# yezhen17/3DIoUMatch

Hardware: AMD Instinct MI355X
Metric: scenes/sec train-step (ScanNet 40k pts, 256 proposals) (higher is better)
Workload: dtype f32

## Files before the change

3dioumatch_amd/csrc/mlp_bwd_fused.hip:

```cpp
#include "common.h"
#include "mlp_operand.h"
#include "mlp_bwd_x6.h"

#ifndef MLP_LIN4_OCC
#define MLP_LIN4_OCC 1
#endif

namespace {

template <int MB, int KB, int KBD, int NB, int PMODE, int QMODE, int OCC, bool STATS, bool DGRAD = true,
          bool X6 = false>
__global__ void __launch_bounds__(256, OCC)
gemm_bwd_fused_kernel(int k_total, int r, int total_chunks, int chunks_per_cloud, int xyz,
                      OperandB opp, OperandB opq, const float *__restrict__ w,
                      float *__restrict__ dq, float *__restrict__ part,
                      float *__restrict__ stats_part) {
  constexpr int M = 32 * MB, KP = 32 * KB, TN = 32 * NB;
  constexpr int LDP = M + 1, LDQ = KP + 1;
  constexpr int TPR = TN / 16;
  constexpr int RPP = 256 / TPR;
  constexpr int PP = (M + RPP - 1) / RPP, QP = (KP + RPP - 1) / RPP;
  constexpr int WMB = MB >= 4 ? MB / 4 : 1;
  constexpr int WKB = MB >= 4 ? KB : KB * MB / 4;
  static_assert(MB >= 4 ? MB % 4 == 0 : (MB == 2 && KB % 2 == 0), "dW blocks must split over 4 waves");
  constexpr int DK = KBD >= 4 ? KBD / 4 : 1;
  constexpr int DN = KBD >= 4 ? NB : 1;
  static_assert(KBD >= 4 ? KBD % 4 == 0 : (KBD == 2 && NB == 2), "dQ blocks must split over 4 waves");
  constexpr int DU = 4, DG = DGRAD ? (X6 ? M / 16 : (M / 2) / DU) : 0;
  constexpr int WU = WMB * WKB >= 4 ? 1 : 2, WG = X6 ? TN / 16 : (TN / 2) / WU;
  constexpr int NS = 4 * (PP + QP), NG = DG + WG;

  __shared__ float Ps[2][TN * LDP];
  __shared__ float Qs[2][TN * LDQ];
  static_assert(DGRAD || !STATS, "the sums come from the dQ blocks");
  static_assert(!STATS || QMODE == OP_BNRELU || QMODE == OP_LIN4,
                "the sums are those of a BatchNorm+ReLU layer below");
  constexpr bool QLIN = QMODE == OP_LIN4;
  static_assert(!QLIN || (STATS && KB * 32 == 64), "recomputed rows: the 64-channel layer only");
  constexpr bool TF = QLIN;
  static_assert(!TF || X6, "the T form is instantiated in the bf16 form only");
  constexpr bool RAWQ = STATS;
  constexpr int SROWS = STATS ? 32 * KBD : 1;
  __shared__ float4 Rc[SROWS];
  __shared__ float4 X4s[TF ? 2 : 1][TF ? TN : 1];
  __shared__ float Wx[3 * M];
  __shared__ float red[8 * 3 * 32];

  const int tid = threadIdx.x, lane = tid & 63, wave = tid >> 6;
  const int l31 = lane & 31, lhi = lane >> 5;
  const int seg_row = tid / TPR, seg_c = (tid % TPR) * 16;
  OperandB P = opp, Q = opq;

  static_assert(M % RPP == 0, "whole passes over the P rows");
  RowCoef pc[PP], qc[QP];
  bool q_ok[QP];
  size_t p_lane[PP], q_lane[QP];
#pragma unroll
  for (int p = 0; p < PP; ++p) {
    pc[p] = load_row_coef<PMODE>(P, seg_row + p * RPP, true);
    p_lane[p] = (size_t)(seg_row + p * RPP) * r + seg_c;
  }
#pragma unroll
  for (int q = 0; q < QP; ++q) {
    const int row = seg_row + q * RPP;
    q_ok[q] = row < k_total;
    qc[q] = load_row_coef<QLIN ? OP_BNRELU : QMODE>(Q, q_ok[q] ? row : k_total - 1, true);
    q_lane[q] = QLIN ? (size_t)seg_c : (size_t)(q_ok[q] ? row : k_total - 1) * r + seg_c;
  }
  float4 qw[QP];
#pragma unroll
  for (int q = 0; q < QP; ++q) {
    const int row = seg_row + q * RPP;
    qw[q] = QLIN && row < k_total ? *reinterpret_cast<const float4 *>(Q.lin_w + (size_t)row * 4)
                                 : make_float4(0.f, 0.f, 0.f, 0.f);
  }
  if (STATS) {
    for (int t = tid; t < SROWS; t += 256)
      Rc[t] = make_float4(Q.scale[t], Q.shift[t], Q.mean[t], Q.invstd[t]);
  }
  float fsc[WKB], fsh[WKB];
#pragma unroll
  for (int j = 0; j < WKB; ++j) {
    const int kb = MB >= 4 ? j : (wave / MB) + (4 / MB) * j;
    const int row = kb * 32 + l31;
    fsc[j] = RAWQ && row < k_total ? Q.scale[row] : 1.f;
    fsh[j] = RAWQ && row < k_total ? Q.shift[row] : 0.f;
  }
  const int lane_g = PMODE == OP_POOLDY ? seg_c / P.ns : 0;
  const int lane_s = PMODE == OP_POOLDY ? seg_c % P.ns : 0;

  float wreg[DK][DGRAD ? M / 2 : 1];
#pragma unroll
  for (int e = 0; e < (DGRAD ? DK : 0); ++e) {
    const int kbd = KBD >= 4 ? wave * DK + e : (wave >> 1);
    const float *wc = w + xyz + 32 * kbd + l31;
#pragma unroll
    for (int s = 0; s < M / 2; ++s)
      wreg[e][s] = wc[(size_t)(X6 ? 16 * (s >> 3) + 8 * lhi + (s & 7) : 2 * s + lhi) * k_total];
  }
  for (int t = tid; t < 3 * M; t += 256) Wx[t] = DGRAD && xyz ? w[(size_t)(t % M) * k_total + t / M] : 0.f;

  f32x16 accW[WMB][WKB];
#pragma unroll
  for (int i = 0; i < WMB; ++i)
#pragma unroll
    for (int j = 0; j < WKB; ++j)
#pragma unroll
      for (int q = 0; q < 16; ++q) accW[i][j][q] = 0.f;

  const int per = (total_chunks + (int)gridDim.x - 1) / (int)gridDim.x;
  const int c_lo = (int)blockIdx.x * per;
  const int c_hi = c_lo + per < total_chunks ? c_lo + per : total_chunks;

  float4 px[PP][4], pd[PP][4], qx[QP][4][QLIN ? 4 : 1];
  int pwin[PP];
  float pdp[PP];
#pragma unroll
  for (int p = 0; p < PP; ++p) {
    pwin[p] = -1; pdp[p] = 0.f;
#pragma unroll
    for (int i = 0; i < 4; ++i) { px[p][i] = make_float4(0.f, 0.f, 0.f, 0.f); pd[p][i] = px[p][i]; }
  }
#pragma unroll
  for (int q = 0; q < QP; ++q)
#pragma unroll
    for (int i = 0; i < 4; ++i)
#pragma unroll
      for (int cc = 0; cc < (QLIN ? 4 : 1); ++cc) qx[q][i][cc] = make_float4(0.f, 0.f, 0.f, 0.f);

  struct ChunkAt { size_t p, q, grp; int s0; };
  auto chunk_at = [&](int c) {
    const int b = c / chunks_per_cloud;
    const int col0 = (c - b * chunks_per_cloud) * TN;
    ChunkAt at;
    at.p = (size_t)b * M * r + col0;
    at.q = (size_t)b * (QLIN ? 4 : k_total) * r + col0;
    at.grp = 0; at.s0 = 0;
    if (PMODE == OP_POOLDY) {
      const int g0 = col0 / P.ns;
      at.grp = (size_t)b * M * P.groups + g0;
      at.s0 = col0 - g0 * P.ns;
    }
    return at;
  };
  auto fetch_slice = [&](int sl, const ChunkAt &at) {
    if (sl < 4 * PP) {
      const int p = sl >> 2, i = sl & 3;
      px[p][i] = *reinterpret_cast<const float4 *>(P.x + at.p + p_lane[p] + 4 * i);
      if (PMODE == OP_DY) {
        pd[p][i] = *reinterpret_cast<const float4 *>(P.dz + at.p + p_lane[p] + 4 * i);
      } else if (PMODE == OP_POOLDY && i == 3) {
        const size_t gi = at.grp + (size_t)(seg_row + p * RPP) * P.groups + lane_g;
        pwin[p] = P.argmax[gi] - (at.s0 + lane_s);
        pdp[p] = P.dz[gi];
      }
    } else {
      const int q = (sl - 4 * PP) >> 2, i = (sl - 4 * PP) & 3;
      if constexpr (QLIN) {
#pragma unroll
        for (int cc = 0; cc < 4; ++cc)
          qx[q][i][cc] = *reinterpret_cast<const float4 *>(Q.x + at.q + (size_t)cc * r + q_lane[q] + 4 * i);
      } else {
        qx[q][i][0] = *reinterpret_cast<const float4 *>(Q.x + at.q + q_lane[q] + 4 * i);
      }
    }
  };
  auto stage_slice = [&](int sl, int buf) {
    if (sl < 4 * PP) {
      const int p = sl >> 2, i = sl & 3;
      const int row = seg_row + p * RPP;
      const float xv[4] = {px[p][i].x, px[p][i].y, px[p][i].z, px[p][i].w};
      const float dv[4] = {pd[p][i].x, pd[p][i].y, pd[p][i].z, pd[p][i].w};
#pragma unroll
      for (int e = 0; e < 4; ++e) {
        const float dz = PMODE == OP_POOLDY ? (4 * i + e == pwin[p] ? pdp[p] : 0.f) : dv[e];
        Ps[buf][(seg_c + 4 * i + e) * LDP + row] = transform<PMODE>(xv[e], dz, pc[p]);
      }
    } else {
      const int q = (sl - 4 * PP) >> 2, i = (sl - 4 * PP) & 3;
      const int row = seg_row + q * RPP;
      if (q * RPP >= KP) return;
      if (KP % RPP != 0 && row >= KP) return;
      float xv[4];
      if constexpr (QLIN) {
        const float c0[4] = {qx[q][i][0].x, qx[q][i][0].y, qx[q][i][0].z, qx[q][i][0].w};
        const float c1[4] = {qx[q][i][1].x, qx[q][i][1].y, qx[q][i][1].z, qx[q][i][1].w};
        const float c2[4] = {qx[q][i][2].x, qx[q][i][2].y, qx[q][i][2].z, qx[q][i][2].w};
        const float c3[4] = {qx[q][i][3].x, qx[q][i][3].y, qx[q][i][3].z, qx[q][i][3].w};
#pragma unroll
        for (int e = 0; e < 4; ++e) xv[e] = lin4(qw[q], c0[e], c1[e], c2[e], c3[e]);
        if (TF && row == 0) {
#pragma unroll
          for (int e = 0; e < 4; ++e) X4s[buf][seg_c + 4 * i + e] = make_float4(c0[e], c1[e], c2[e], c3[e]);
        }
      } else {
        xv[0] = qx[q][i][0].x; xv[1] = qx[q][i][0].y; xv[2] = qx[q][i][0].z; xv[3] = qx[q][i][0].w;
      }
#pragma unroll
      for (int e = 0; e < 4; ++e)
        Qs[buf][(seg_c + 4 * i + e) * LDQ + row] =
            q_ok[q] ? (RAWQ ? xv[e] : transform<QLIN ? OP_BNRELU : QMODE>(xv[e], 0.f, qc[q])) : 0.f;
    }
  };

  constexpr int SQ = (STATS && !TF) ? 16 : 1;
  float st1[DK][SQ], st2[DK][SQ];
  float gx[TF ? DK : 1][4];
#pragma unroll
  for (int e = 0; e < (TF ? DK : 1); ++e)
#pragma unroll
    for (int k = 0; k < 4; ++k) gx[e][k] = 0.f;
  float4 trc[TF ? DK : 1];
#pragma unroll
  for (int e = 0; e < (TF ? DK : 1); ++e) {
    const int row = 32 * (KBD >= 4 ? wave * DK + e : (wave >> 1)) + l31;
    trc[e] = TF ? make_float4(Q.scale[row], Q.shift[row], Q.mean[row], Q.invstd[row]) : make_float4(0.f, 0.f, 0.f, 0.f);
  }
#pragma unroll
  for (int e = 0; e < DK; ++e)
#pragma unroll
    for (int q = 0; q < SQ; ++q) { st1[e][q] = 0.f; st2[e][q] = 0.f; }

  if (c_lo < c_hi) {
    const ChunkAt first = chunk_at(c_lo), second = chunk_at(c_lo + 1 < c_hi ? c_lo + 1 : c_lo);
#pragma unroll
    for (int sl = 0; sl < NS; ++sl) fetch_slice(sl, first);
#pragma unroll
    for (int sl = 0; sl < NS; ++sl) {
      stage_slice(sl, 0);
      fetch_slice(sl, second);
    }
  }
  __syncthreads();

  for (int c = c_lo; c < c_hi; ++c) {
    const int cur = (c - c_lo) & 1;
    const float *Pc = Ps[cur], *Qc = Qs[cur];
    const ChunkAt ahead = chunk_at(c + 2 < c_hi ? c + 2 : c_hi - 1);
    auto between = [&](int g) {
#if !defined(BWDF_ABL) || BWDF_ABL != 1
#pragma unroll
      for (int sl = g * NS / NG; sl < (g + 1) * NS / NG; ++sl) {
        stage_slice(sl, cur ^ 1);
        fetch_slice(sl, ahead);
      }
#endif
    };
    const int b = c / chunks_per_cloud;
    const int col0 = (c - b * chunks_per_cloud) * TN;

    f32x16 accD[DK][DN];
    if (DGRAD) {
#pragma unroll
      for (int e = 0; e < DK; ++e)
#pragma unroll
        for (int n = 0; n < DN; ++n)
#pragma unroll
          for (int q = 0; q < 16; ++q) accD[e][n][q] = 0.f;
      if constexpr (X6) {
        float bp8[DN][8];
        auto frag8 = [&](int g) {
#pragma unroll
          for (int n = 0; n < DN; ++n) {
            const int nb = KBD >= 4 ? n : (wave & 1);
#pragma unroll
            for (int j = 0; j < 8; ++j) bp8[n][j] = Pc[(nb * 32 + l31) * LDP + 16 * g + 8 * lhi + j];
          }
        };
        frag8(0);
#pragma unroll
        for (int g = 0; g < DG; ++g) {
          Split3 sb[DN];
#pragma unroll
          for (int n = 0; n < DN; ++n) sb[n] = split3(bp8[n]);
          if (g + 1 < DG) frag8(g + 1);
#pragma unroll
          for (int e = 0; e < DK; ++e) {
            float w8[8];
#pragma unroll
            for (int j = 0; j < 8; ++j) w8[j] = wreg[e][g * 8 + j];
            const Split3 sa = split3(w8);
#pragma unroll
            for (int n = 0; n < DN; ++n) {
              if constexpr (TF) mfma_x6(accD[e][n], sb[n], sa);
              else mfma_x6(accD[e][n], sa, sb[n]);
            }
          }
          between(g);
        }
      } else {
      float bp[2][DU][DN];
      auto frag = [&](int g, float (&dst)[DU][DN]) {
#pragma unroll
        for (int u = 0; u < DU; ++u)
#pragma unroll
          for (int n = 0; n < DN; ++n) {
            const int nb = KBD >= 4 ? n : (wave & 1);
            dst[u][n] = Pc[(nb * 32 + l31) * LDP + 2 * (g * DU + u) + lhi];
          }
      };
      frag(0, bp[0]);
#pragma unroll
      for (int g = 0; g < DG; ++g) {
        if (g + 1 < DG) frag(g + 1, bp[(g + 1) & 1]);
        __builtin_amdgcn_sched_barrier(0);
#pragma unroll
        for (int u = 0; u < DU; ++u)
#pragma unroll
          for (int e = 0; e < DK; ++e)
#pragma unroll
            for (int n = 0; n < DN; ++n)
              accD[e][n] = __builtin_amdgcn_mfma_f32_32x32x2f32(wreg[e][g * DU + u], bp[g & 1][u][n],
                                                                accD[e][n], 0, 0, 0);
        between(g);
        __builtin_amdgcn_sched_barrier(0);
      }
      }
#pragma unroll
      for (int e = 0; e < (TF ? 0 : DK); ++e) {
        const int kbd = KBD >= 4 ? wave * DK + e : (wave >> 1);
#pragma unroll
        for (int n = 0; n < DN; ++n) {
          const int nb = KBD >= 4 ? n : (wave & 1);
          float *dst = dq + ((size_t)b * k_total + xyz + 32 * kbd + 4 * lhi) * r + col0 + nb * 32 + l31;
#pragma unroll
          for (int q = 0; q < 16; ++q)
            __builtin_nontemporal_store(accD[e][n][q], &dst[(size_t)((q & 3) + 8 * (q >> 2)) * r]);
        }
      }
    }

    auto stats_row = [&](int q) {
      const int ro = (q & 3) + 8 * (q >> 2);
      if constexpr (TF) {
#pragma unroll
        for (int e = 0; e < DK; ++e) {
          const int kbd = KBD >= 4 ? wave * DK + e : (wave >> 1);
#pragma unroll
          for (int n = 0; n < DN; ++n) {
            const int nb = KBD >= 4 ? n : (wave & 1);
            const int col = nb * 32 + 4 * lhi + ro;
            const float yv = Qc[col * LDQ + 32 * kbd + l31];
            const float g = __fmaf_rn(yv, trc[e].x, trc[e].y) > 0.f ? accD[e][n][q] : 0.f;
            st1[e][0] += g;
            st2[e][0] = __fmaf_rn(g, (yv - trc[e].z) * trc[e].w, st2[e][0]);
            const float4 xc = X4s[cur][col];
            gx[e][0] = __fmaf_rn(g, xc.x, gx[e][0]);
            gx[e][1] = __fmaf_rn(g, xc.y, gx[e][1]);
            gx[e][2] = __fmaf_rn(g, xc.z, gx[e][2]);
            gx[e][3] = __fmaf_rn(g, xc.w, gx[e][3]);
          }
        }
        return;
      }
#pragma unroll
      for (int e = 0; e < DK; ++e) {
        const int kbd = KBD >= 4 ? wave * DK + e : (wave >> 1);
        const float4 rc = Rc[32 * kbd + 4 * lhi + ro];
#pragma unroll
        for (int n = 0; n < DN; ++n) {
          const int nb = KBD >= 4 ? n : (wave & 1);
          const float yv = Qc[(nb * 32 + l31) * LDQ + 32 * kbd + 4 * lhi + ro];
          const float g = __fmaf_rn(yv, rc.x, rc.y) > 0.f ? accD[e][n][q] : 0.f;
          st1[e][STATS ? q : 0] += g;
          st2[e][STATS ? q : 0] = __fmaf_rn(g, (yv - rc.z) * rc.w, st2[e][STATS ? q : 0]);
        }
      }
    };
    if constexpr (X6) {
      float qraw[8];
      auto qfrag = [&](int g, int j) {
        const int kb = MB >= 4 ? j : (wave / MB) + (4 / MB) * j;
#pragma unroll
        for (int jj = 0; jj < 8; ++jj) {
          const float raw = Qc[(16 * g + 8 * lhi + jj) * LDQ + kb * 32 + l31];
          qraw[jj] = RAWQ ? fmaxf(__fmaf_rn(raw, fsc[j], fsh[j]), 0.f) : raw;
        }
      };
#pragma unroll
      for (int g = 0; g < WG; ++g) {
        Split3 sp[WMB];
#pragma unroll
        for (int i = 0; i < WMB; ++i) {
          const int mb = MB >= 4 ? wave + 4 * i : wave % MB;
          float praw[8];
#pragma unroll
          for (int jj = 0; jj < 8; ++jj) praw[jj] = Pc[(16 * g + 8 * lhi + jj) * LDP + mb * 32 + l31];
          sp[i] = split3(praw);
        }
        qfrag(g, 0);
#pragma unroll
        for (int j = 0; j < WKB; ++j) {
          const Split3 sq = split3(qraw);
          if (j + 1 < WKB) qfrag(g, j + 1);
#pragma unroll
          for (int i = 0; i < WMB; ++i) mfma_x6(accW[i][j], sp[i], sq);
        }
        between(DG + g);
        if (STATS) {
#pragma unroll
          for (int q = g * 16 / WG; q < (g + 1) * 16 / WG; ++q) stats_row(q);
        }
      }
    } else {
      float ap[2][WU][WMB], bq[2][WU][WKB];
      auto frag = [&](int g, float (&a)[WU][WMB], float (&bb)[WU][WKB]) {
#pragma unroll
        for (int u = 0; u < WU; ++u) {
          const int n = 2 * (g * WU + u) + lhi;
#pragma unroll
          for (int i = 0; i < WMB; ++i) {
            const int mb = MB >= 4 ? wave + 4 * i : wave % MB;
            a[u][i] = Pc[n * LDP + mb * 32 + l31];
          }
#pragma unroll
          for (int j = 0; j < WKB; ++j) {
            const int kb = MB >= 4 ? j : (wave / MB) + (4 / MB) * j;
            const float raw = Qc[n * LDQ + kb * 32 + l31];
            bb[u][j] = RAWQ ? fmaxf(__fmaf_rn(raw, fsc[j], fsh[j]), 0.f) : raw;
          }
        }
      };
      frag(0, ap[0], bq[0]);
#pragma unroll
      for (int g = 0; g < WG; ++g) {
        if (g + 1 < WG) frag(g + 1, ap[(g + 1) & 1], bq[(g + 1) & 1]);
        __builtin_amdgcn_sched_barrier(0);
#pragma unroll
        for (int u = 0; u < WU; ++u)
#pragma unroll
          for (int i = 0; i < WMB; ++i)
#pragma unroll
            for (int j = 0; j < WKB; ++j)
              accW[i][j] = __builtin_amdgcn_mfma_f32_32x32x2f32(ap[g & 1][u][i], bq[g & 1][u][j],
                                                                accW[i][j], 0, 0, 0);
        between(DG + g);
        if (STATS) {
#pragma unroll
          for (int q = g * 16 / WG; q < (g + 1) * 16 / WG; ++q) stats_row(q);
        }
        __builtin_amdgcn_sched_barrier(0);
      }
    }

    if (DGRAD && NB == 1 && xyz) {
      const int n = tid & 31, g8 = tid >> 5;
      float s0 = 0.f, s1 = 0.f, s2 = 0.f;
#pragma unroll 4
      for (int mm = g8 * (M / 8); mm < (g8 + 1) * (M / 8); ++mm) {
        const float pv = Pc[n * LDP + mm];
        s0 = __fmaf_rn(pv, Wx[mm], s0);
        s1 = __fmaf_rn(pv, Wx[M + mm], s1);
        s2 = __fmaf_rn(pv, Wx[2 * M + mm], s2);
      }
      red[(g8 * 3 + 0) * 32 + n] = s0;
      red[(g8 * 3 + 1) * 32 + n] = s1;
      red[(g8 * 3 + 2) * 32 + n] = s2;
      __syncthreads();
      if (tid < 96) {
        const int kx = tid >> 5;
        float t = 0.f;
#pragma unroll
        for (int g = 0; g < 8; ++g) t += red[(g * 3 + kx) * 32 + n];
        dq[((size_t)b * k_total + kx) * r + col0 + n] = t;
      }
    }
    __syncthreads();
  }

  if constexpr (TF) {
    constexpr int PPW = KBD >= 4 ? 1 : 2;
    const int parts = (int)gridDim.x * PPW;
    const int pidx = (int)blockIdx.x * PPW + (KBD >= 4 ? 0 : (wave & 1));
#pragma unroll
    for (int e = 0; e < DK; ++e) {
      const int row = 32 * (KBD >= 4 ? wave * DK + e : (wave >> 1)) + l31;
      float a1 = st1[e][0], a2 = st2[e][0];
      a1 += __shfl_xor(a1, 32, kWave);
      a2 += __shfl_xor(a2, 32, kWave);
      float g4[4];
#pragma unroll
      for (int k = 0; k < 4; ++k) g4[k] = gx[e][k] + __shfl_xor(gx[e][k], 32, kWave);
      if (lhi == 0) {
        if (stats_part != nullptr) {
          stats_part[((size_t)row * parts + pidx) * 2] = a1;
          stats_part[((size_t)row * parts + pidx) * 2 + 1] = a2;
        }
        *reinterpret_cast<float4 *>(dq + ((size_t)pidx * k_total + row) * 4) = make_float4(g4[0], g4[1], g4[2], g4[3]);
      }
    }
  } else if (STATS && stats_part != nullptr) {
    constexpr int PPW = KBD >= 4 ? 1 : 2;
    const int parts = (int)gridDim.x * PPW;
    const int pidx = (int)blockIdx.x * PPW + (KBD >= 4 ? 0 : (wave & 1));
#pragma unroll
    for (int e = 0; e < DK; ++e) {
      const int kbd = KBD >= 4 ? wave * DK + e : (wave >> 1);
#pragma unroll
      for (int q = 0; q < SQ; ++q) {
        float a1 = st1[e][q], a2 = st2[e][q];
#pragma unroll
        for (int off = 1; off < 32; off <<= 1) {
          a1 += __shfl_xor(a1, off, kWave);
          a2 += __shfl_xor(a2, off, kWave);
        }
        if (l31 == 0) {
          const int row = 32 * kbd + 4 * lhi + (q & 3) + 8 * (q >> 2);
          stats_part[((size_t)row * parts + pidx) * 2] = a1;
          stats_part[((size_t)row * parts + pidx) * 2 + 1] = a2;
        }
      }
    }
  }
  float *out = part + (size_t)blockIdx.x * M * k_total;
#pragma unroll
  for (int i = 0; i < WMB; ++i) {
    const int mb = MB >= 4 ? wave + 4 * i : wave % MB;
#pragma unroll
    for (int j = 0; j < WKB; ++j) {
      const int kb = MB >= 4 ? j : (wave / MB) + (4 / MB) * j;
      const int colk = kb * 32 + l31;
      if (colk >= k_total) continue;
#pragma unroll
      for (int q = 0; q < 16; ++q) {
        const int row = mb * 32 + (q & 3) + 8 * (q >> 2) + 4 * lhi;
        out[(size_t)row * k_total + colk] = accW[i][j][q];
      }
    }
  }
}

struct FusedShape { int m, k, xyz, tn, occ; };

bool fused_shape(int m, int k, FusedShape *s) {
  static const FusedShape table[] = {
      {64, 64, 0, 64, 2}, {128, 64, 0, 64, 1}, {128, 128, 0, 32, 2},
      {256, 128, 0, 32, 1}, {128, 131, 3, 32, 1}, {128, 259, 3, 32, 1},
  };
  for (const FusedShape &t : table)
    if (t.m == m && t.k == k) { *s = t; return true; }
  return false;
}

int fused_workgroups(const FusedShape &s, long long total_chunks) {
  long long g = (long long)pn2_cu_count() * s.occ;
  if (g > total_chunks / 8) g = total_chunks / 8;
  return (int)(g < 1 ? 1 : g);
}

}

#define MLP_API extern "C" __attribute__((visibility("default")))

MLP_API int mlp_gemm_backward_fused_supported(int b, int m, int k, int r, int pmode, int qmode,
                                              int ns) {
  FusedShape s;
  if (b <= 0 || r <= 0 || !fused_shape(m, k, &s)) return 0;
  if (r % s.tn != 0 || (long long)b * (r / s.tn) < 64) return 0;
  if (pmode != OP_DY && pmode != OP_POOLDY) return 0;
  if (pmode == OP_POOLDY && (ns <= 0 || ns % 16 != 0 || r % ns != 0 || (ns % s.tn != 0 && s.tn % ns != 0)))
    return 0;
  if (qmode == OP_LIN4) return m == 64 && k == 64 && pmode == OP_DY;
  const bool first = s.xyz != 0;
  if (first != (qmode == OP_DIRECT)) return 0;
  if (qmode != OP_DIRECT && qmode != OP_BNRELU) return 0;
  const bool pooled_only = (m == 128 && k == 64) || (m == 256 && k == 128);
  const bool either = m == 128 && k == 128;
  if (!either && pooled_only != (pmode == OP_POOLDY)) return 0;
  return 1;
}

MLP_API int mlp_gemm_backward_fused_stats_parts(int b, int m, int k, int r) {
  FusedShape s;
  const int gx = mlp_bwd_x6_workgroups(b, m, k, r, pn2_cu_count());
  if (gx > 0) return gx;
  if (!fused_shape(m, k, &s) || k != 64 || r % s.tn != 0) return 0;
  return fused_workgroups(s, (long long)b * (r / s.tn)) * 2;
}

MLP_API size_t mlp_gemm_backward_fused_workspace_floats(int b, int m, int k, int r) {
  FusedShape s;
  if (!fused_shape(m, k, &s) || r % s.tn != 0) return 0;
  const long long g0 = fused_workgroups(s, (long long)b * (r / s.tn));
  const long long g1 = mlp_bwd_x6_workgroups(b, m, k, r, pn2_cu_count());
  return (size_t)(g0 > g1 ? g0 : g1) * m * k;
}

MLP_API int mlp_gemm_backward_fused(int b, int m, int k, int r, const float *w, const MlpOperand *dy,
                                    const MlpOperand *x, float *dq, float *dw, float *workspace,
                                    float *stats_part, void *stream_) {
  if (b <= 0 || m <= 0 || k <= 0 || r <= 0) return 0;
  OperandB P, Q;
  int orc = operand_from_abi(dy, op_bit(OP_DY) | op_bit(OP_POOLDY), r, &P);
  if (!orc) orc = operand_from_abi(x, op_bit(OP_DIRECT) | op_bit(OP_BNRELU) | op_bit(OP_LIN4), r, &Q);
  if (orc) return orc;
  const int pmode = dy->mode, qmode = x->mode;
  if (qmode != OP_DIRECT && (!Q.mean || !Q.invstd)) return (int)hipErrorInvalidValue;
  if (!mlp_gemm_backward_fused_supported(b, m, k, r, pmode, qmode, P.ns)) return (int)hipErrorInvalidValue;
  FusedShape s;
  fused_shape(m, k, &s);
  if (dq == nullptr && !(m == 128 && k == 259)) return (int)hipErrorInvalidValue;
  hipStream_t stream = (hipStream_t)stream_;
  const int cpc = r / s.tn;
  const int total = b * cpc;
  const int g = fused_workgroups(s, total);
  {
    int gx = 0;
    const int rcx = mlp_bwd_x6_try(b, m, k, r, pmode, qmode, P, Q, w, dq, workspace,
                                   qmode == OP_BNRELU ? stats_part : nullptr, pn2_cu_count(), &gx, stream);
    if (rcx > 0) return rcx;
    if (rcx == 0) return mlp_reduce_weight_partials(m * k, gx, workspace, dw, stream);
  }
  if (k != 64) stats_part = nullptr;
#define FUSED_X(MB, KB, KBD, NB, PM, QM, OCC, ST, X6)                                           \
  hipLaunchKernelGGL((gemm_bwd_fused_kernel<MB, KB, KBD, NB, PM, QM, OCC, ST, true, X6>), dim3(g), \
                     dim3(256), 0, stream, k, r, total, cpc, s.xyz, P, Q, w, dq, workspace,     \
                     stats_part)
#define FUSED(MB, KB, KBD, NB, PM, QM, OCC, ST) FUSED_X(MB, KB, KBD, NB, PM, QM, OCC, ST, true)
#define FUSED_F32(MB, KB, KBD, NB, PM, QM, OCC, ST) FUSED_X(MB, KB, KBD, NB, PM, QM, OCC, ST, false)
  if (m == 64 && k == 64 && qmode == OP_LIN4) FUSED(2, 2, 2, 2, OP_DY, OP_LIN4, MLP_LIN4_OCC, true);
  else if (m == 64 && k == 64) FUSED(2, 2, 2, 2, OP_DY, OP_BNRELU, 2, true);
  else if (m == 128 && k == 64) FUSED(4, 2, 2, 2, OP_POOLDY, OP_BNRELU, 1, true);
  else if (m == 256 && k == 128) FUSED(8, 4, 4, 1, OP_POOLDY, OP_BNRELU, 1, false);
  else if (m == 128 && k == 131) FUSED(4, 5, 4, 1, OP_DY, OP_DIRECT, 1, false);
  else if (dq != nullptr) FUSED_F32(4, 9, 8, 1, OP_DY, OP_DIRECT, 1, false);
  else
    hipLaunchKernelGGL((gemm_bwd_fused_kernel<4, 9, 8, 1, OP_DY, OP_DIRECT, 1, false, false, true>), dim3(g),
                       dim3(256), 0, stream, k, r, total, cpc, s.xyz, P, Q, w, dq, workspace, stats_part);
#undef FUSED_F32
#undef FUSED
#undef FUSED_X
  int rc = pn2_launch_status();
  if (rc) return rc;
  return mlp_reduce_weight_partials(m * k, g, workspace, dw, stream);
}
```

Before: 1407.

## Split LIN4 backward into a warp-specialized 512-thread kernel with data/weight roles

Moves the 64x64 LIN4 layer's backward out of the generic fused kernel into a dedicated 512-thread kernel. Four waves compute the data gradient, BatchNorm statistics and the xyz gradient, while the other four compute the weight gradient in parallel. The two roles share double-buffered LDS tiles and split the eight staging slices between them via a compile-time bitmask. This is meant to overlap the dW and dQ MFMA work that one wave group previously did in sequence, at the cost of doubled threads per block and occupancy fixed at 1.

```diff
diff --git a/3dioumatch_amd/csrc/mlp_bwd_fused.hip b/3dioumatch_amd/csrc/mlp_bwd_fused.hip
--- a/3dioumatch_amd/csrc/mlp_bwd_fused.hip
+++ b/3dioumatch_amd/csrc/mlp_bwd_fused.hip
@@ -1,10 +1,6 @@
 #include "common.h"
 #include "mlp_operand.h"
 #include "mlp_bwd_x6.h"
-
-#ifndef MLP_LIN4_OCC
-#define MLP_LIN4_OCC 1
-#endif
 
 namespace {
 
@@ -33,16 +29,10 @@
   __shared__ float Ps[2][TN * LDP];
   __shared__ float Qs[2][TN * LDQ];
   static_assert(DGRAD || !STATS, "the sums come from the dQ blocks");
-  static_assert(!STATS || QMODE == OP_BNRELU || QMODE == OP_LIN4,
-                "the sums are those of a BatchNorm+ReLU layer below");
-  constexpr bool QLIN = QMODE == OP_LIN4;
-  static_assert(!QLIN || (STATS && KB * 32 == 64), "recomputed rows: the 64-channel layer only");
-  constexpr bool TF = QLIN;
-  static_assert(!TF || X6, "the T form is instantiated in the bf16 form only");
+  static_assert(!STATS || QMODE == OP_BNRELU, "the sums are those of a BatchNorm+ReLU layer below");
   constexpr bool RAWQ = STATS;
   constexpr int SROWS = STATS ? 32 * KBD : 1;
   __shared__ float4 Rc[SROWS];
-  __shared__ float4 X4s[TF ? 2 : 1][TF ? TN : 1];
   __shared__ float Wx[3 * M];
   __shared__ float red[8 * 3 * 32];
 
@@ -64,15 +54,8 @@
   for (int q = 0; q < QP; ++q) {
     const int row = seg_row + q * RPP;
     q_ok[q] = row < k_total;
-    qc[q] = load_row_coef<QLIN ? OP_BNRELU : QMODE>(Q, q_ok[q] ? row : k_total - 1, true);
-    q_lane[q] = QLIN ? (size_t)seg_c : (size_t)(q_ok[q] ? row : k_total - 1) * r + seg_c;
-  }
-  float4 qw[QP];
-#pragma unroll
-  for (int q = 0; q < QP; ++q) {
-    const int row = seg_row + q * RPP;
-    qw[q] = QLIN && row < k_total ? *reinterpret_cast<const float4 *>(Q.lin_w + (size_t)row * 4)
-                                 : make_float4(0.f, 0.f, 0.f, 0.f);
+    qc[q] = load_row_coef<QMODE>(Q, q_ok[q] ? row : k_total - 1, true);
+    q_lane[q] = (size_t)(q_ok[q] ? row : k_total - 1) * r + seg_c;
   }
   if (STATS) {
     for (int t = tid; t < SROWS; t += 256)
@@ -112,7 +95,7 @@
   const int c_lo = (int)blockIdx.x * per;
   const int c_hi = c_lo + per < total_chunks ? c_lo + per : total_chunks;
 
-  float4 px[PP][4], pd[PP][4], qx[QP][4][QLIN ? 4 : 1];
+  float4 px[PP][4], pd[PP][4], qx[QP][4];
   int pwin[PP];
   float pdp[PP];
 #pragma unroll
@@ -124,9 +107,7 @@
 #pragma unroll
   for (int q = 0; q < QP; ++q)
 #pragma unroll
-    for (int i = 0; i < 4; ++i)
-#pragma unroll
-      for (int cc = 0; cc < (QLIN ? 4 : 1); ++cc) qx[q][i][cc] = make_float4(0.f, 0.f, 0.f, 0.f);
+    for (int i = 0; i < 4; ++i) qx[q][i] = make_float4(0.f, 0.f, 0.f, 0.f);
 
   struct ChunkAt { size_t p, q, grp; int s0; };
   auto chunk_at = [&](int c) {
@@ -134,7 +115,7 @@
     const int col0 = (c - b * chunks_per_cloud) * TN;
     ChunkAt at;
     at.p = (size_t)b * M * r + col0;
-    at.q = (size_t)b * (QLIN ? 4 : k_total) * r + col0;
+    at.q = (size_t)b * k_total * r + col0;
     at.grp = 0; at.s0 = 0;
     if (PMODE == OP_POOLDY) {
       const int g0 = col0 / P.ns;
@@ -156,13 +137,7 @@
       }
     } else {
       const int q = (sl - 4 * PP) >> 2, i = (sl - 4 * PP) & 3;
-      if constexpr (QLIN) {
-#pragma unroll
-        for (int cc = 0; cc < 4; ++cc)
-          qx[q][i][cc] = *reinterpret_cast<const float4 *>(Q.x + at.q + (size_t)cc * r + q_lane[q] + 4 * i);
-      } else {
-        qx[q][i][0] = *reinterpret_cast<const float4 *>(Q.x + at.q + q_lane[q] + 4 * i);
-      }
+      qx[q][i] = *reinterpret_cast<const float4 *>(Q.x + at.q + q_lane[q] + 4 * i);
     }
   };
   auto stage_slice = [&](int sl, int buf) {
@@ -181,41 +156,16 @@
       const int row = seg_row + q * RPP;
       if (q * RPP >= KP) return;
       if (KP % RPP != 0 && row >= KP) return;
-      float xv[4];
-      if constexpr (QLIN) {
-        const float c0[4] = {qx[q][i][0].x, qx[q][i][0].y, qx[q][i][0].z, qx[q][i][0].w};
-        const float c1[4] = {qx[q][i][1].x, qx[q][i][1].y, qx[q][i][1].z, qx[q][i][1].w};
-        const float c2[4] = {qx[q][i][2].x, qx[q][i][2].y, qx[q][i][2].z, qx[q][i][2].w};
-        const float c3[4] = {qx[q][i][3].x, qx[q][i][3].y, qx[q][i][3].z, qx[q][i][3].w};
-#pragma unroll
-        for (int e = 0; e < 4; ++e) xv[e] = lin4(qw[q], c0[e], c1[e], c2[e], c3[e]);
-        if (TF && row == 0) {
-#pragma unroll
-          for (int e = 0; e < 4; ++e) X4s[buf][seg_c + 4 * i + e] = make_float4(c0[e], c1[e], c2[e], c3[e]);
-        }
-      } else {
-        xv[0] = qx[q][i][0].x; xv[1] = qx[q][i][0].y; xv[2] = qx[q][i][0].z; xv[3] = qx[q][i][0].w;
-      }
+      const float xv[4] = {qx[q][i].x, qx[q][i].y, qx[q][i].z, qx[q][i].w};
 #pragma unroll
       for (int e = 0; e < 4; ++e)
         Qs[buf][(seg_c + 4 * i + e) * LDQ + row] =
-            q_ok[q] ? (RAWQ ? xv[e] : transform<QLIN ? OP_BNRELU : QMODE>(xv[e], 0.f, qc[q])) : 0.f;
+            q_ok[q] ? (RAWQ ? xv[e] : transform<QMODE>(xv[e], 0.f, qc[q])) : 0.f;
     }
   };
 
-  constexpr int SQ = (STATS && !TF) ? 16 : 1;
+  constexpr int SQ = STATS ? 16 : 1;
   float st1[DK][SQ], st2[DK][SQ];
-  float gx[TF ? DK : 1][4];
-#pragma unroll
-  for (int e = 0; e < (TF ? DK : 1); ++e)
-#pragma unroll
-    for (int k = 0; k < 4; ++k) gx[e][k] = 0.f;
-  float4 trc[TF ? DK : 1];
-#pragma unroll
-  for (int e = 0; e < (TF ? DK : 1); ++e) {
-    const int row = 32 * (KBD >= 4 ? wave * DK + e : (wave >> 1)) + l31;
-    trc[e] = TF ? make_float4(Q.scale[row], Q.shift[row], Q.mean[row], Q.invstd[row]) : make_float4(0.f, 0.f, 0.f, 0.f);
-  }
 #pragma unroll
   for (int e = 0; e < DK; ++e)
 #pragma unroll
@@ -281,10 +231,7 @@
             for (int j = 0; j < 8; ++j) w8[j] = wreg[e][g * 8 + j];
             const Split3 sa = split3(w8);
 #pragma unroll
-            for (int n = 0; n < DN; ++n) {
-              if constexpr (TF) mfma_x6(accD[e][n], sb[n], sa);
-              else mfma_x6(accD[e][n], sa, sb[n]);
-            }
+            for (int n = 0; n < DN; ++n) mfma_x6(accD[e][n], sa, sb[n]);
           }
           between(g);
         }
@@ -317,7 +264,7 @@
       }
       }
 #pragma unroll
-      for (int e = 0; e < (TF ? 0 : DK); ++e) {
+      for (int e = 0; e < DK; ++e) {
         const int kbd = KBD >= 4 ? wave * DK + e : (wave >> 1);
 #pragma unroll
         for (int n = 0; n < DN; ++n) {
@@ -332,27 +279,6 @@
 
     auto stats_row = [&](int q) {
       const int ro = (q & 3) + 8 * (q >> 2);
-      if constexpr (TF) {
-#pragma unroll
-        for (int e = 0; e < DK; ++e) {
-          const int kbd = KBD >= 4 ? wave * DK + e : (wave >> 1);
-#pragma unroll
-          for (int n = 0; n < DN; ++n) {
-            const int nb = KBD >= 4 ? n : (wave & 1);
-            const int col = nb * 32 + 4 * lhi + ro;
-            const float yv = Qc[col * LDQ + 32 * kbd + l31];
-            const float g = __fmaf_rn(yv, trc[e].x, trc[e].y) > 0.f ? accD[e][n][q] : 0.f;
-            st1[e][0] += g;
-            st2[e][0] = __fmaf_rn(g, (yv - trc[e].z) * trc[e].w, st2[e][0]);
-            const float4 xc = X4s[cur][col];
-            gx[e][0] = __fmaf_rn(g, xc.x, gx[e][0]);
-            gx[e][1] = __fmaf_rn(g, xc.y, gx[e][1]);
-            gx[e][2] = __fmaf_rn(g, xc.z, gx[e][2]);
-            gx[e][3] = __fmaf_rn(g, xc.w, gx[e][3]);
-          }
-        }
-        return;
-      }
 #pragma unroll
       for (int e = 0; e < DK; ++e) {
         const int kbd = KBD >= 4 ? wave * DK + e : (wave >> 1);
@@ -468,28 +394,7 @@
     __syncthreads();
   }
 
-  if constexpr (TF) {
-    constexpr int PPW = KBD >= 4 ? 1 : 2;
-    const int parts = (int)gridDim.x * PPW;
-    const int pidx = (int)blockIdx.x * PPW + (KBD >= 4 ? 0 : (wave & 1));
-#pragma unroll
-    for (int e = 0; e < DK; ++e) {
-      const int row = 32 * (KBD >= 4 ? wave * DK + e : (wave >> 1)) + l31;
-      float a1 = st1[e][0], a2 = st2[e][0];
-      a1 += __shfl_xor(a1, 32, kWave);
-      a2 += __shfl_xor(a2, 32, kWave);
-      float g4[4];
-#pragma unroll
-      for (int k = 0; k < 4; ++k) g4[k] = gx[e][k] + __shfl_xor(gx[e][k], 32, kWave);
-      if (lhi == 0) {
-        if (stats_part != nullptr) {
-          stats_part[((size_t)row * parts + pidx) * 2] = a1;
-          stats_part[((size_t)row * parts + pidx) * 2 + 1] = a2;
-        }
-        *reinterpret_cast<float4 *>(dq + ((size_t)pidx * k_total + row) * 4) = make_float4(g4[0], g4[1], g4[2], g4[3]);
-      }
-    }
-  } else if (STATS && stats_part != nullptr) {
+  if (STATS && stats_part != nullptr) {
     constexpr int PPW = KBD >= 4 ? 1 : 2;
     const int parts = (int)gridDim.x * PPW;
     const int pidx = (int)blockIdx.x * PPW + (KBD >= 4 ? 0 : (wave & 1));
@@ -528,6 +433,237 @@
       }
     }
   }
+}
+
+#ifndef BWDF_LIN4_DATA_SLICES
+#define BWDF_LIN4_DATA_SLICES 0xF0u
+#endif
+static_assert((BWDF_LIN4_DATA_SLICES & ~0xFFu) == 0u, "eight slices: the table is eight bits");
+
+struct Lin4Tiles {
+  float Ps[2][64 * 65];
+  float Qs[2][64 * 65];
+  float4 X4s[2][64];
+};
+
+template <bool DATA>
+__device__ __forceinline__ void gemm_bwd_lin4_role(int r, int total_chunks, int chunks_per_cloud,
+                                                   const OperandB &P, const OperandB &Q,
+                                                   const float *__restrict__ w, float *__restrict__ gpart,
+                                                   float *__restrict__ part, float *__restrict__ stats_part,
+                                                   Lin4Tiles &lds, int tid, int wave) {
+  constexpr int M = 64, K = 64, TN = 64, LD = 65;
+  constexpr int DG = M / 16, WG = TN / 16;
+  constexpr int NS = 8;
+  constexpr unsigned MINE = (DATA ? BWDF_LIN4_DATA_SLICES : ~BWDF_LIN4_DATA_SLICES) & 0xFFu;
+  constexpr int NOWN = x6_popcount(MINE);
+  constexpr int NG = DATA ? DG : WG;
+#define LIN4_MINE(sl) (((MINE >> (sl)) & 1u) != 0u)
+
+  const int lane = tid & 63;
+  const int l31 = lane & 31, lhi = lane >> 5;
+  const int seg_row = tid >> 2, seg_c = (tid & 3) * 16;
+
+  const RowCoef pc = load_row_coef<OP_DY>(P, seg_row, true);
+  const size_t p_lane = (size_t)seg_row * r + seg_c;
+  const float4 qw = *reinterpret_cast<const float4 *>(Q.lin_w + (size_t)seg_row * 4);
+
+  const int mb = wave & 1, kb = wave >> 1;
+  const float fsc = DATA ? 1.f : Q.scale[kb * 32 + l31], fsh = DATA ? 0.f : Q.shift[kb * 32 + l31];
+  f32x16 accW;
+#pragma unroll
+  for (int q = 0; q < 16; ++q) accW[q] = 0.f;
+
+  const int kbd = wave >> 1, nbd = wave & 1;
+  float wreg[DATA ? M / 2 : 1];
+  float st1 = 0.f, st2 = 0.f, gx[4] = {0.f, 0.f, 0.f, 0.f};
+  float4 trc = make_float4(0.f, 0.f, 0.f, 0.f);
+  if constexpr (DATA) {
+    const float *wc = w + 32 * kbd + l31;
+#pragma unroll
+    for (int s = 0; s < M / 2; ++s) wreg[s] = wc[(size_t)(16 * (s >> 3) + 8 * lhi + (s & 7)) * K];
+    const int row = 32 * kbd + l31;
+    trc = make_float4(Q.scale[row], Q.shift[row], Q.mean[row], Q.invstd[row]);
+  }
+
+  const int per = (total_chunks + (int)gridDim.x - 1) / (int)gridDim.x;
+  const int c_lo = (int)blockIdx.x * per;
+  const int c_hi = c_lo + per < total_chunks ? c_lo + per : total_chunks;
+
+  float4 px[4], pd[4], qx[4][4];
+#pragma unroll
+  for (int i = 0; i < 4; ++i) {
+    px[i] = make_float4(0.f, 0.f, 0.f, 0.f); pd[i] = px[i];
+#pragma unroll
+    for (int cc = 0; cc < 4; ++cc) qx[i][cc] = px[i];
+  }
+
+  struct ChunkAt { size_t p, q; };
+  auto chunk_at = [&](int c) {
+    const int b = c / chunks_per_cloud;
+    const int col0 = (c - b * chunks_per_cloud) * TN;
+    ChunkAt at;
+    at.p = (size_t)b * M * r + col0;
+    at.q = (size_t)b * 4 * r + col0;
+    return at;
+  };
+  auto fetch_slice = [&](int sl, const ChunkAt &at) {
+    const int i = sl & 3;
+    if (sl < 4) {
+      px[i] = *reinterpret_cast<const float4 *>(P.x + at.p + p_lane + 4 * i);
+      pd[i] = *reinterpret_cast<const float4 *>(P.dz + at.p + p_lane + 4 * i);
+    } else {
+#pragma unroll
+      for (int cc = 0; cc < 4; ++cc)
+        qx[i][cc] = *reinterpret_cast<const float4 *>(Q.x + at.q + (size_t)cc * r + seg_c + 4 * i);
+    }
+  };
+  auto stage_slice = [&](int sl, int buf) {
+    const int i = sl & 3;
+    if (sl < 4) {
+      const float xv[4] = {px[i].x, px[i].y, px[i].z, px[i].w};
+      const float dv[4] = {pd[i].x, pd[i].y, pd[i].z, pd[i].w};
+#pragma unroll
+      for (int e = 0; e < 4; ++e) lds.Ps[buf][(seg_c + 4 * i + e) * LD + seg_row] = transform<OP_DY>(xv[e], dv[e], pc);
+    } else {
+      const float c0[4] = {qx[i][0].x, qx[i][0].y, qx[i][0].z, qx[i][0].w};
+      const float c1[4] = {qx[i][1].x, qx[i][1].y, qx[i][1].z, qx[i][1].w};
+      const float c2[4] = {qx[i][2].x, qx[i][2].y, qx[i][2].z, qx[i][2].w};
+      const float c3[4] = {qx[i][3].x, qx[i][3].y, qx[i][3].z, qx[i][3].w};
+#pragma unroll
+      for (int e = 0; e < 4; ++e)
+        lds.Qs[buf][(seg_c + 4 * i + e) * LD + seg_row] = lin4(qw, c0[e], c1[e], c2[e], c3[e]);
+      if (seg_row == 0) {
+#pragma unroll
+        for (int e = 0; e < 4; ++e) lds.X4s[buf][seg_c + 4 * i + e] = make_float4(c0[e], c1[e], c2[e], c3[e]);
+      }
+    }
+  };
+
+  auto clampc = [&](int c) { return c < c_hi ? c : c_hi - 1; };
+  if (c_lo < c_hi) {
+    const ChunkAt first = chunk_at(c_lo), second = chunk_at(clampc(c_lo + 1));
+#pragma unroll
+    for (int sl = 0; sl < NS; ++sl)
+      if (LIN4_MINE(sl)) fetch_slice(sl, first);
+#pragma unroll
+    for (int sl = 0; sl < NS; ++sl) {
+      if (!LIN4_MINE(sl)) continue;
+      stage_slice(sl, 0);
+      fetch_slice(sl, second);
+    }
+  }
+  __syncthreads();
+
+  for (int c = c_lo; c < c_hi; ++c) {
+    const int cur = (c - c_lo) & 1;
+    const float *Pc = lds.Ps[cur], *Qc = lds.Qs[cur];
+    const ChunkAt ahead = chunk_at(clampc(c + 2));
+    auto between = [&](int g) {
+      int own = 0;
+#pragma unroll
+      for (int sl = 0; sl < NS; ++sl) {
+        if (!LIN4_MINE(sl)) continue;
+        if (own >= g * NOWN / NG && own < (g + 1) * NOWN / NG) {
+          stage_slice(sl, cur ^ 1);
+          fetch_slice(sl, ahead);
+        }
+        ++own;
+      }
+    };
+
+    if constexpr (DATA) {
+      f32x16 accD;
+#pragma unroll
+      for (int q = 0; q < 16; ++q) accD[q] = 0.f;
+      float bp8[8];
+      auto frag8 = [&](int g) {
+#pragma unroll
+        for (int j = 0; j < 8; ++j) bp8[j] = Pc[(nbd * 32 + l31) * LD + 16 * g + 8 * lhi + j];
+      };
+      frag8(0);
+#pragma unroll
+      for (int g = 0; g < DG; ++g) {
+        const Split3 sb = split3(bp8);
+        if (g + 1 < DG) frag8(g + 1);
+        float w8[8];
+#pragma unroll
+        for (int j = 0; j < 8; ++j) w8[j] = wreg[g * 8 + j];
+        const Split3 sa = split3(w8);
+        mfma_x6(accD, sb, sa);
+        between(g);
+      }
+#pragma unroll
+      for (int q = 0; q < 16; ++q) {
+        const int col = nbd * 32 + 4 * lhi + (q & 3) + 8 * (q >> 2);
+        const float yv = Qc[col * LD + 32 * kbd + l31];
+        const float g = __fmaf_rn(yv, trc.x, trc.y) > 0.f ? accD[q] : 0.f;
+        st1 += g;
+        st2 = __fmaf_rn(g, (yv - trc.z) * trc.w, st2);
+        const float4 xc = lds.X4s[cur][col];
+        gx[0] = __fmaf_rn(g, xc.x, gx[0]);
+        gx[1] = __fmaf_rn(g, xc.y, gx[1]);
+        gx[2] = __fmaf_rn(g, xc.z, gx[2]);
+        gx[3] = __fmaf_rn(g, xc.w, gx[3]);
+      }
+    } else {
+#pragma unroll
+      for (int g = 0; g < WG; ++g) {
+        float praw[8], qraw[8];
+#pragma unroll
+        for (int jj = 0; jj < 8; ++jj) praw[jj] = Pc[(16 * g + 8 * lhi + jj) * LD + mb * 32 + l31];
+        const Split3 sp = split3(praw);
+#pragma unroll
+        for (int jj = 0; jj < 8; ++jj)
+          qraw[jj] = fmaxf(__fmaf_rn(Qc[(16 * g + 8 * lhi + jj) * LD + kb * 32 + l31], fsc, fsh), 0.f);
+        const Split3 sq = split3(qraw);
+        mfma_x6(accW, sp, sq);
+        between(g);
+      }
+    }
+    __syncthreads();
+  }
+
+  if constexpr (DATA) {
+    const int parts = (int)gridDim.x * 2;
+    const int pidx = (int)blockIdx.x * 2 + nbd;
+    const int row = 32 * kbd + l31;
+    float a1 = st1, a2 = st2;
+    a1 += __shfl_xor(a1, 32, kWave);
+    a2 += __shfl_xor(a2, 32, kWave);
+    float g4[4];
+#pragma unroll
+    for (int k = 0; k < 4; ++k) g4[k] = gx[k] + __shfl_xor(gx[k], 32, kWave);
+    if (lhi == 0) {
+      if (stats_part != nullptr) {
+        stats_part[((size_t)row * parts + pidx) * 2] = a1;
+        stats_part[((size_t)row * parts + pidx) * 2 + 1] = a2;
+      }
+      *reinterpret_cast<float4 *>(gpart + ((size_t)pidx * K + row) * 4) = make_float4(g4[0], g4[1], g4[2], g4[3]);
+    }
+  } else {
+    float *out = part + (size_t)blockIdx.x * M * K;
+#pragma unroll
+    for (int q = 0; q < 16; ++q) {
+      const int row = mb * 32 + (q & 3) + 8 * (q >> 2) + 4 * lhi;
+      out[(size_t)row * K + kb * 32 + l31] = accW[q];
+    }
+  }
+#undef LIN4_MINE
+}
+
+__global__ void __launch_bounds__(512, 1)
+gemm_bwd_lin4_kernel(int r, int total_chunks, int chunks_per_cloud, OperandB opp, OperandB opq,
+                     const float *__restrict__ w, float *__restrict__ gpart, float *__restrict__ part,
+                     float *__restrict__ stats_part) {
+  __shared__ Lin4Tiles lds;
+  const int wave = __builtin_amdgcn_readfirstlane((int)threadIdx.x >> 6);
+  if (wave < 4)
+    gemm_bwd_lin4_role<true>(r, total_chunks, chunks_per_cloud, opp, opq, w, gpart, part, stats_part, lds,
+                             (int)threadIdx.x, wave);
+  else
+    gemm_bwd_lin4_role<false>(r, total_chunks, chunks_per_cloud, opp, opq, w, gpart, part, stats_part, lds,
+                              (int)threadIdx.x - 256, wave - 4);
 }
 
 struct FusedShape { int m, k, xyz, tn, occ; };
@@ -618,7 +754,9 @@
                      stats_part)
 #define FUSED(MB, KB, KBD, NB, PM, QM, OCC, ST) FUSED_X(MB, KB, KBD, NB, PM, QM, OCC, ST, true)
 #define FUSED_F32(MB, KB, KBD, NB, PM, QM, OCC, ST) FUSED_X(MB, KB, KBD, NB, PM, QM, OCC, ST, false)
-  if (m == 64 && k == 64 && qmode == OP_LIN4) FUSED(2, 2, 2, 2, OP_DY, OP_LIN4, MLP_LIN4_OCC, true);
+  if (m == 64 && k == 64 && qmode == OP_LIN4)
+    hipLaunchKernelGGL(gemm_bwd_lin4_kernel, dim3(g), dim3(512), 0, stream, r, total, cpc, P, Q, w, dq, workspace,
+                       stats_part);
   else if (m == 64 && k == 64) FUSED(2, 2, 2, 2, OP_DY, OP_BNRELU, 2, true);
   else if (m == 128 && k == 64) FUSED(4, 2, 2, 2, OP_POOLDY, OP_BNRELU, 1, true);
   else if (m == 256 && k == 128) FUSED(8, 4, 4, 1, OP_POOLDY, OP_BNRELU, 1, false);
```

Result: no change. 1420, median of 5 (+0.9%).
